# Ced3-han/PepFlowww

Measured on AMD Instinct MI355X. Metric: residues x denoise-steps / s, higher is better.
Workload: dtype f32 (fp32 storage and accumulation; matrix products as 3 x f16 split MFMA, ~22-bit operands); 1 GPU; cfg4/GPU: B=64 x 128-residue synthetic pockets (112 ctx + 16 gen) per GPU; per_gpu_batch=64, residues=128, global_batch=64, parallelism=batch-shard x1, hipgraph=True, precision=fp32

## Files before the change

pepflowww_amd/csrc/ipa_split.hip:

```cpp
#include <cstdlib>
#include <type_traits>
#include "common.h"
#include "../../include/pepflow_hip.h"

#ifdef PF_PROFILE
__device__ long long g_prof_ipas[64];
#define PROFS(i) do { if (blockIdx.x == gridDim.x / 2 + 3 && threadIdx.x == 64) g_prof_ipas[i] = clock64(); } while (0)
extern "C" int pf_debug_prof_ipas(long long* out, int n) {
    return (int)hipMemcpyFromSymbol(out, HIP_SYMBOL(g_prof_ipas), sizeof(long long) * n, 0, hipMemcpyDeviceToHost);
}
#else
#define PROFS(i)
#endif

namespace {

typedef float f32x2 __attribute__((ext_vector_type(2)));
constexpr int H = PF_HEADS, C = PF_C_HID, PQ = PF_QK_PTS, PV = PF_V_PTS;
constexpr int OFF_KV = 1024;
#ifndef PF_IPA_WMAX
#define PF_IPA_WMAX 8
#endif
constexpr int WMAX = PF_IPA_WMAX;
constexpr int KPS = 28;
constexpr int VPS = 36;

__device__ __forceinline__ float softplusf2(float x) { return x > 20.f ? x : log1pf(expf(x)); }

template <bool D16> struct DzVec { typedef float4 type; };
template <> struct DzVec<true> { typedef half4 type; };

template <int NB4, bool D16>
__device__ __forceinline__ void pair_dz_rows(const void* __restrict__ dzp, size_t rowb, int L, int i0, int Le, int kt,
                                             const float* __restrict__ Pw, int SLD, int ks, int cq, f32x2 (&acc)[32]) {
    typedef typename DzVec<D16>::type V4;
    typedef typename std::conditional<D16, _Float16, float>::type DT;
    constexpr int NT = 4 * NB4;
    const DT* base = reinterpret_cast<const DT*>(dzp) + rowb * (size_t)L * 16 + 4 * cq;
    int koff[NT];
    float on[NT];
#pragma unroll
    for (int u = 0; u < NT; ++u) {
        const int uu = min(u, kt - 1);
        koff[u] = min(16 * uu + ks, L - 1) * 16;
        on[u] = u < kt ? 1.f : 0.f;
    }
    auto load_row = [&](int qi, V4 (&buf)[NT]) {
        const DT* row = base + (size_t)min(i0 + qi, Le - 1) * L * 16;
#pragma unroll
        for (int u = 0; u < NT; ++u) buf[u] = *reinterpret_cast<const V4*>(row + koff[u]);
    };
    auto mac_row = [&](int qi, const V4 (&buf)[NT]) {
        const float* pr = Pw + qi * SLD;
#pragma unroll
        for (int u = 0; u < NT; ++u) {
            float pv;
            if (u <= 4 * (NB4 - 1)) pv = pr[16 * u];
            else pv = pr[16 * min(u, kt - 1)] * on[u];
            const f32x2 p2 = {pv, pv};
            f32x2 d0, d1;
            if constexpr (D16) { d0 = (f32x2){(float)buf[u][0], (float)buf[u][1]}; d1 = (f32x2){(float)buf[u][2], (float)buf[u][3]}; }
            else { d0 = (f32x2){buf[u].x, buf[u].y}; d1 = (f32x2){buf[u].z, buf[u].w}; }
            acc[2 * qi] = __builtin_elementwise_fma(d0, p2, acc[2 * qi]);
            acc[2 * qi + 1] = __builtin_elementwise_fma(d1, p2, acc[2 * qi + 1]);
        }
    };
    constexpr int D = NB4 == 1 ? 8 : NB4 == 2 ? 4 : 2;
    V4 buf[D][NT];
#pragma unroll
    for (int d = 0; d < D - 1; ++d) load_row(d, buf[d]);
#pragma unroll
    for (int qi = 0; qi < 16; ++qi) {
        load_row(min(qi + D - 1, 15), buf[(qi + D - 1) % D]);
        __builtin_amdgcn_sched_barrier(0);
        mac_row(qi, buf[qi % D]);
        __builtin_amdgcn_sched_barrier(0);
    }
}

template <bool D16>
__device__ __forceinline__ void pair_dz_phase(const pf_ipa_attn_args& a, size_t rowb, int h, int i0, int Le, int kt, const float* Pwave,
                                              int SLD, float inv, int lane) {
    const int ks = (lane & 3) | ((lane >> 4) << 2), cq = (lane >> 2) & 3;
    f32x2 acc[32];
#pragma unroll
    for (int k = 0; k < 32; ++k) acc[k] = (f32x2){0.f, 0.f};
    const float* Pw = Pwave + ks;
    const int nb4 = (kt + 3) >> 2;
    if (nb4 <= 1) pair_dz_rows<1, D16>(a.dz, rowb, a.L, i0, Le, kt, Pw, SLD, ks, cq, acc);
    else if (nb4 == 2) pair_dz_rows<2, D16>(a.dz, rowb, a.L, i0, Le, kt, Pw, SLD, ks, cq, acc);
    else if (nb4 == 3) pair_dz_rows<3, D16>(a.dz, rowb, a.L, i0, Le, kt, Pw, SLD, ks, cq, acc);
    else pair_dz_rows<4, D16>(a.dz, rowb, a.L, i0, Le, kt, Pw, SLD, ks, cq, acc);
    float v[64];
#pragma unroll
    for (int k = 0; k < 32; ++k) { v[2 * k] = acc[k][0]; v[2 * k + 1] = acc[k][1]; }
    float w[32], x[16], y[8], z4[4];
#pragma unroll
    for (int k = 0; k < 32; ++k) {
        auto rr = __builtin_amdgcn_permlane32_swap(__float_as_uint(v[k]), __float_as_uint(v[k + 32]), false, false);
        w[k] = __uint_as_float(rr[0]) + __uint_as_float(rr[1]);
    }
#pragma unroll
    for (int k = 0; k < 16; ++k) {
        auto rr = __builtin_amdgcn_permlane16_swap(__float_as_uint(w[k]), __float_as_uint(w[k + 16]), false, false);
        x[k] = __uint_as_float(rr[0]) + __uint_as_float(rr[1]);
    }
    {
        const bool hi = lane & 2;
#pragma unroll
        for (int k = 0; k < 8; ++k) {
            const float send = hi ? x[k] : x[k + 8], keep = hi ? x[k + 8] : x[k];
            y[k] = keep + lane_xor2(send);
        }
    }
    {
        const bool hi = lane & 1;
#pragma unroll
        for (int k = 0; k < 4; ++k) {
            const float send = hi ? y[k] : y[k + 4], keep = hi ? y[k + 4] : y[k];
            z4[k] = keep + lane_xor1(send);
        }
    }
    const int qi = ((lane >> 5) & 1) * 8 + ((lane >> 4) & 1) * 4 + (lane & 3);
    const float invq = __shfl(inv, qi);
    const float4 bd = *reinterpret_cast<const float4*>(a.b_dz + 4 * cq);
    const int i = min(i0 + qi, Le - 1);
    *reinterpret_cast<float4*>(a.feats + (rowb + i) * PF_IPA_FEATS + 1408 + h * 16 + 4 * cq) =
        make_float4(z4[0] * invq + bd.x, z4[1] * invq + bd.y, z4[2] * invq + bd.z, z4[3] * invq + bd.w);
}

template <int I, int N, class F> __device__ __forceinline__ void cfor_p(F&& f) {
    if constexpr (I < N) {
        f(std::integral_constant<int, I>{});
        cfor_p<I + 1, N>(f);
    }
}
constexpr int PJ_TILES = 31;
constexpr int PJ_NPAD = 3968;
constexpr int PJ_CT = 3;
constexpr int PJ_NCH = (PJ_TILES + PJ_CT - 1) / PJ_CT;
constexpr int PJ_CHUNK_B = PJ_CT * 8 * 1024;
constexpr int PJ_NB = 4;
constexpr int PJ_STAGE_B = PJ_NB * PJ_CHUNK_B;
__device__ __forceinline__ constexpr int pj_tile(int idx, int h) {
    return idx < 8 ? 8 * h + idx : idx < 24 ? 64 + 16 * h + (idx - 8) : idx < 26 ? 192 + 2 * h + (idx - 24) : 208 + 5 * h + (idx - 26);
}
__device__ __forceinline__ void pj_glds16(const void* sbase, unsigned voff, unsigned lds_addr) {
    const unsigned long long v = (unsigned long long)sbase;
    const unsigned lo = __builtin_amdgcn_readfirstlane((unsigned)v), hi = __builtin_amdgcn_readfirstlane((unsigned)(v >> 32));
    const void* sb = (const void*)(((unsigned long long)hi << 32) | lo);
    lds_addr = __builtin_amdgcn_readfirstlane(lds_addr);
    asm volatile("s_mov_b32 m0, %2\n\ts_nop 4\n\tglobal_load_lds_dwordx4 %0, %1" : : "v"(voff), "s"(sb), "s"(lds_addr) : "memory", "m0");
}
template <int N> __device__ __forceinline__ void pj_wait_vm() { asm volatile("s_waitcnt vmcnt(%0)" : : "n"(N) : "memory"); }
__device__ __forceinline__ void pj_wait_vm_dyn(int n) {
    n = __builtin_amdgcn_readfirstlane(n);
    switch (n > 40 ? 40 : n) {
#define PJ_W(k) case k: pj_wait_vm<k>(); break;
        PJ_W(0) PJ_W(1) PJ_W(2) PJ_W(3) PJ_W(4) PJ_W(5) PJ_W(6) PJ_W(7) PJ_W(8) PJ_W(9) PJ_W(10) PJ_W(11) PJ_W(12) PJ_W(13) PJ_W(14)
        PJ_W(15) PJ_W(16) PJ_W(17) PJ_W(18) PJ_W(19) PJ_W(20) PJ_W(21) PJ_W(22) PJ_W(23) PJ_W(24) PJ_W(25) PJ_W(26) PJ_W(27) PJ_W(28)
        PJ_W(29) PJ_W(30) PJ_W(31) PJ_W(32) PJ_W(33) PJ_W(34) PJ_W(35) PJ_W(36) PJ_W(37) PJ_W(38) PJ_W(39) PJ_W(40)
#undef PJ_W
    }
}
__device__ __forceinline__ constexpr int pj_vt_row(int f) { return f < 64 ? 16 * (f & 3) + (f >> 2) : 64 + 16 * ((f - 64) & 3) + ((f - 64) >> 2); }
__device__ __forceinline__ int pj_vt_pos(int j) { return (j & ~31) + 8 * ((j >> 2) & 3) + 4 * ((j >> 4) & 1) + (j & 3); }
__host__ __device__ __forceinline__ constexpr int pj_vtl(int LP) { return ((LP + 31) & ~31) + 8; }
__host__ __device__ __forceinline__ constexpr int pj_vp_floats(int LP) {
    return LP * VPS > 48 * pj_vtl(LP) ? LP * VPS : 48 * pj_vtl(LP);
}
struct PjW { half8 h[4], l[4]; };
template <bool KF> __device__ __forceinline__ constexpr int pj_ntiles() { return KF ? PJ_TILES - 8 : PJ_TILES; }
template <bool KF> __device__ __forceinline__ constexpr int pj_nch() { return (pj_ntiles<KF>() + PJ_CT - 1) / PJ_CT; }
template <bool KF> __device__ __forceinline__ constexpr int pj_orig(int j) { return KF && j >= 8 ? j + 8 : j; }
__device__ __forceinline__ constexpr bool pj_q_tile(int idx) { return idx < 8 || idx == 24 || idx == 25; }
template <bool KS, bool KF = false>
__device__ __forceinline__ void proj_head(const pf_ipa_attn_args& a, size_t rowb, int iq, int h, int jrow, int LPe, bool wave_on, int role, int tile, float* KP,
                                          _Float16* VPT , int VTL, _Float16* VTH , int VTG,
                                          unsigned char* WS , float* QPW ,
                                          float* PB ,
                                          float4 (&qf)[8], float4 (&qp4)[6], int lane, int wave, int nw) {
    const int r = lane & 15, g = lane >> 4;
    PROFS(8);
    const unsigned char* whp = reinterpret_cast<const unsigned char*>(a.proj_w_f16);
    const unsigned char* wlp = whp + (size_t)PJ_NPAD * 128 * 2;
    const unsigned ws0 = (unsigned)(size_t)(__attribute__((address_space(3))) void*)WS;
    const unsigned l16 = lane * 16;
    const int ppw = (PJ_CT * 8 + nw - 1) / nw;
    constexpr int NT = pj_ntiles<KF>(), NCH = pj_nch<KF>();
    auto issue = [&](int c) __attribute__((always_inline)) {
        const int npc = min(PJ_CT, NT - PJ_CT * c) * 8;
        for (int k = 0; k < ppw; ++k) {
            const int pc = min(wave + k * nw, npc - 1);
            const int tl = pc >> 3, ks = (pc >> 1) & 3, pl = pc & 1;
            const int T16 = pj_tile(pj_orig<KF>(PJ_CT * c + tl), h);
            pj_glds16((pl ? wlp : whp) + (size_t)(T16 * 4 + ks) * 1024, l16, ws0 + (c % PJ_NB) * PJ_CHUNK_B + pc * 1024);
        }
    };
    for (int i = wave * 64 + lane; i < PJ_TILES * 16; i += nw * 64) PB[i] = a.proj_bias[16 * pj_tile(i >> 4, h) + (i & 15)];
    for (int i = wave * 64 + lane; i < 24 * VTL; i += nw * 64) reinterpret_cast<float2*>(VPT)[i] = make_float2(0.f, 0.f);
    PROFS(30);
    half8 xh[4], xl[4];
    float R[9], T[3];
    {
        const float* xrow = a.s_in + (rowb + iq) * 128 + 8 * g;
        float4 t[8];
#pragma unroll
        for (int ks = 0; ks < 4; ++ks) { t[2 * ks] = *reinterpret_cast<const float4*>(xrow + 32 * ks); t[2 * ks + 1] = *reinterpret_cast<const float4*>(xrow + 32 * ks + 4); }
        const float* Rg = a.rot + (rowb + iq) * 9;
        const float* Tg = a.trans + (rowb + iq) * 3;
#pragma unroll
        for (int k = 0; k < 9; ++k) R[k] = Rg[k];
#pragma unroll
        for (int k = 0; k < 3; ++k) T[k] = Tg[k];
#pragma unroll
        for (int ks = 0; ks < 4; ++ks) {
            const float v0[4] = {t[2 * ks].x, t[2 * ks].y, t[2 * ks].z, t[2 * ks].w}, v1[4] = {t[2 * ks + 1].x, t[2 * ks + 1].y, t[2 * ks + 1].z, t[2 * ks + 1].w};
            half4 h0, l0, h1, l1;
            split4(v0, h0, l0);
            split4(v1, h1, l1);
#pragma unroll
            for (int e = 0; e < 4; ++e) { xh[ks][e] = h0[e]; xh[ks][4 + e] = h1[e]; xl[ks][e] = l0[e]; xl[ks][4 + e] = l1[e]; }
        }
    }
    PROFS(31);
    if constexpr (KF && !KS) {
        float* kfrag32 = reinterpret_cast<float*>(VTH + (size_t)8 * (VTG >> 5) * 1024 + (size_t)tile * 4096);
        if (wave_on && role != 1) {
            const float* krow = a.s_in + (rowb + iq) * 128 + 4 * g;
#pragma unroll
            for (int hb = 0; hb < 2; ++hb) {
                float4 kt[4];
#pragma unroll
                for (int u = 0; u < 4; ++u) kt[u] = *reinterpret_cast<const float4*>(krow + 16 * (4 * hb + u));
#pragma unroll
                for (int u = 0; u < 4; ++u) *reinterpret_cast<float4*>(kfrag32 + (4 * hb + u) * 256 + lane * 4) = kt[u];
            }
        }
    }
    PROFS(32);
    asm volatile("" ::: "memory");
#pragma unroll
    for (int c = 0; c < PJ_NB - 1; ++c)
        if (c < NCH) issue(c);
    PROFS(33);
    _Float16* kfrag = VTH + (size_t)8 * (VTG >> 5) * 1024 + (size_t)tile * 4096 + lane * 8;
    float qpr[2][3] = {{0.f, 0.f, 0.f}, {0.f, 0.f, 0.f}};
    auto ldfrag = [&](int c, int tl, PjW& w) __attribute__((always_inline)) {
        const unsigned char* b = WS + (c % PJ_NB) * PJ_CHUNK_B + tl * 8192 + lane * 16;
#pragma unroll
        for (int ks = 0; ks < 4; ++ks) {
            w.h[ks] = *reinterpret_cast<const half8*>(b + ks * 2048);
            w.l[ks] = *reinterpret_cast<const half8*>(b + ks * 2048 + 1024);
        }
    };
    cfor_p<0, NCH>([&](auto ic) __attribute__((always_inline)) {
        constexpr int c = decltype(ic)::value;
        constexpr int NDY = (c + 1 < NCH) + (PJ_NB > 3 && c + 2 < NCH) + (PJ_NB > 4 && c + 3 < NCH);
        static_assert(PJ_NB == 2 || PJ_NB == 4, "wait accounting written for 2 or 4 staging buffers");
        PROFS(9 + 2 * c);
        pj_wait_vm_dyn(PJ_NB == 2 ? 0 : NDY * ppw);
        if constexpr (c == 0) asm volatile("s_waitcnt lgkmcnt(0)" ::: "memory");
        __builtin_amdgcn_s_barrier();
        PROFS(10 + 2 * c);
        asm volatile("" ::: "memory");
        if constexpr (c + PJ_NB - 1 < NCH) issue(c + PJ_NB - 1);
        if (wave_on) {
            PjW wa, wb;
            if (role == 0) ldfrag(c, 0, wa);
            cfor_p<0, PJ_CT>([&](auto it) __attribute__((always_inline)) {
                constexpr int tl = decltype(it)::value, jt = PJ_CT * c + tl, idx = pj_orig<KF>(jt);
                if constexpr (jt < NT) {
                  if (role == 0 || (role == 1) == pj_q_tile(idx)) {
                    PjW& w = (tl & 1) ? wb : wa;
                    if (role != 0) ldfrag(c, tl, w);
                    else if constexpr (tl + 1 < PJ_CT && jt + 1 < NT) ldfrag(c, tl + 1, (tl & 1) ? wa : wb);
                    constexpr bool VTILE = idx >= 16 && idx < 24;
                    f32x4 am = {0.f, 0.f, 0.f, 0.f}, ac = {0.f, 0.f, 0.f, 0.f};
#pragma unroll
                    for (int ks = 0; ks < 4; ++ks) {
                        if constexpr (VTILE) {
                            am = mfma_h(xh[ks], w.h[ks], am);
                            ac = mfma_h(xl[ks], w.h[ks], ac);
                            ac = mfma_h(xh[ks], w.l[ks], ac);
                        } else {
                            am = mfma_h(w.h[ks], xh[ks], am);
                            ac = mfma_h(w.h[ks], xl[ks], ac);
// ... 224 lines not shown
                for (int cc = 0; cc < 3; ++cc) qv[3 * (4 * t2 + gs) + cc] = __shfl(qpr[t2][cc], r + 16 * gs, 64);
#pragma unroll
        for (int q = 0; q < 6; ++q) qp4[q] = make_float4(qv[4 * q], qv[4 * q + 1], qv[4 * q + 2], qv[4 * q + 3]);
    }
}

template <bool VEC4, bool FUSE = false, bool PROJ = false, bool KFRAG = false, bool KF = false, bool HELP = true>
__global__ __launch_bounds__(512) void ipa_scores_kernel(pf_ipa_attn_args a, int nrb, int rows_per_block, int LP, int SLD, unsigned kfs_b ) {
    extern __shared__ __attribute__((aligned(16))) float smem[];
    constexpr bool KSPLIT = PROJ && !FUSE;
    const int L = a.L;
    float* KP = smem;
    float* MJ = KP + LP * KPS;
    float* VP = MJ + LP;
    float* SW = VP + (PROJ ? pj_vp_floats(LP) : LP * VPS);

    const int tid = threadIdx.x, wave = tid >> 6, lane = tid & 63;
    const int r = lane & 15, g = lane >> 4;
    const int lid = xcd_remap(blockIdx.x, gridDim.x);
    const int rb = lid % nrb;
    const int h = (lid / nrb) % H;
    const int b = lid / (nrb * H);
    const size_t rowb = (size_t)b * L;
    const int ntq = rows_per_block >> 4;
    const bool helper = PROJ && HELP && wave >= ntq;
    const int i0 = rb * rows_per_block + (helper ? wave - ntq : wave) * 16;
    const int Le = a.key_end ? min(__builtin_amdgcn_readfirstlane(a.key_end[b]), L) : L;
    const int kt = (Le + 15) >> 4, ktf = Le >> 4;
    const bool wave_on = i0 < Le;
    if (rb * rows_per_block >= Le) return;
    const int LPe = 16 * kt;
    PROFS(0);

    const int iq = max(min(i0 + r, Le - 1), 0);
    float4 qf[8];
    float4 qp4[6];
    if constexpr (!PROJ) {
        const float* qrow = a.proj + (rowb + iq) * a.ldp + h * C + 4 * g;
#pragma unroll
        for (int s = 0; s < 8; ++s) qf[s] = *reinterpret_cast<const float4*>(qrow + 16 * s);
#pragma unroll
        for (int q = 0; q < 6; ++q) qp4[q] = *reinterpret_cast<const float4*>(a.qp + (rowb + iq) * 192 + h * 24 + 4 * q);
    }
    const float mi = a.mask[rowb + iq];
    const float gamma = softplusf2(a.head_w[h]) * 0.09622504486493763f;
    const float* kbase = a.proj + rowb * a.ldp + OFF_KV + h * 2 * C + 4 * g;
    const char* kfr_u = nullptr;
    if constexpr (KSPLIT && KF) {
        kfr_u = reinterpret_cast<const char*>(a.k_frag_s) + (size_t)b * kfs_b;
    } else if constexpr (PROJ) {
        const int VTG = (L + 31) & ~31;
        kfr_u = reinterpret_cast<const char*>(a.att_vt) + (((size_t)b * H + h) * 512 * VTG + (size_t)8 * (VTG >> 5) * 1024) * sizeof(_Float16);
    }
    auto loadk = [&](int t, float4 (&kf)[8]) {
        if constexpr (KSPLIT) {
            const char* kt_u = kfr_u + (size_t)t * 8192;
#pragma unroll
            for (int s = 0; s < 4; ++s) {
                kf[s] = *reinterpret_cast<const float4*>(kt_u + s * 2048 + (unsigned)lane * 16u);
                kf[4 + s] = *reinterpret_cast<const float4*>(kt_u + s * 2048 + 1024 + (unsigned)lane * 16u);
            }
        } else if constexpr (PROJ) {
            const char* kt_u = kfr_u + (size_t)t * 8192;
#pragma unroll
            for (int s = 0; s < 8; ++s) kf[s] = *reinterpret_cast<const float4*>(kt_u + s * 1024 + (unsigned)lane * 16u);
        } else if constexpr (KFRAG) {
            const float* kt_f = a.k_frag + ((((size_t)b * H + h) * (L >> 4) + t) * 8) * 256 + lane * 4;
#pragma unroll
            for (int s = 0; s < 8; ++s) kf[s] = *reinterpret_cast<const float4*>(kt_f + s * 256);
        } else {
            const float* krow = kbase + (size_t)min(16 * t + r, Le - 1) * a.ldp;
#pragma unroll
            for (int s = 0; s < 8; ++s) kf[s] = *reinterpret_cast<const float4*>(krow + 16 * s);
        }
    };
    float4 kf[8], kn[8];
    half8 qh[4], ql[4];
    if constexpr (!PROJ) { if (wave_on) loadk(0, kf); }

    if constexpr (PROJ) {
        for (int j = tid; j < LPe; j += blockDim.x) MJ[j] = j < L ? a.mask[rowb + min(j, L - 1)] : 0.f;
        unsigned char* WS = reinterpret_cast<unsigned char*>(SW);
        float* QPW = reinterpret_cast<float*>(WS + PJ_STAGE_B) + (helper ? 0 : wave) * 16 * 24;
        float* PB = reinterpret_cast<float*>(WS + PJ_STAGE_B) + ntq * 16 * 24;
        const int role = HELP ? ((int)(blockDim.x >> 6) > ntq ? (helper ? 2 : 1) : 0) : 0;
        const int VTG = (L + 31) & ~31;
        _Float16* VTH = reinterpret_cast<_Float16*>(const_cast<void*>(a.att_vt)) + ((size_t)b * H + h) * 512 * VTG;
        proj_head<KSPLIT, KF>(a, rowb, iq, h, i0 + r, LPe, wave_on, role, helper ? wave - ntq : wave, KP, reinterpret_cast<_Float16*>(VP), pj_vtl(LP), VTH, VTG, WS, QPW,
                  PB, qf, qp4, lane, wave, (int)(blockDim.x >> 6));
        __syncthreads();
        if (!wave_on || helper) return;
        loadk(0, kf);
#pragma unroll
        for (int s = 0; KSPLIT && s < 4; ++s) {
            const float v[8] = {qf[2 * s].x, qf[2 * s].y, qf[2 * s].z, qf[2 * s].w, qf[2 * s + 1].x, qf[2 * s + 1].y, qf[2 * s + 1].z, qf[2 * s + 1].w};
#pragma unroll
            for (int j = 0; j < 8; ++j) qh[s][j] = (_Float16)v[j];
            pf_pin(qh[s]);
#pragma unroll
            for (int j = 0; j < 8; ++j) ql[s][j] = (_Float16)(v[j] - (float)qh[s][j]);
        }
    } else {
    {
        const int nth = blockDim.x;
        constexpr int KB = 2, VB = 3;
        float4 k4[KB], v4[VB];
        float mj0 = 0.f;
#pragma unroll
        for (int u = 0; u < KB; ++u) {
            const int idx = min(tid + u * nth, LPe * 6 - 1), j = idx / 6, q = idx - j * 6;
            k4[u] = *reinterpret_cast<const float4*>(a.kp + (rowb + min(j, L - 1)) * 192 + h * 24 + 4 * q);
        }
        mj0 = a.mask[rowb + min(tid, L - 1)];
        mj0 = tid < L ? mj0 : 0.f;
#pragma unroll
        for (int u = 0; u < VB; ++u) {
            const int idx = min(tid + u * nth, LPe * 9 - 1), j = idx / 9, q = idx - j * 9;
            v4[u] = *reinterpret_cast<const float4*>(a.vp + (rowb + min(j, L - 1)) * 288 + h * 36 + 4 * q);
        }
        asm volatile("" : "+v"(k4[0].x), "+v"(k4[0].y), "+v"(k4[0].z), "+v"(k4[0].w), "+v"(k4[1].x), "+v"(k4[1].y), "+v"(k4[1].z), "+v"(k4[1].w), "+v"(mj0));
        asm volatile("" : "+v"(v4[0].x), "+v"(v4[0].y), "+v"(v4[0].z), "+v"(v4[0].w), "+v"(v4[1].x), "+v"(v4[1].y), "+v"(v4[1].z), "+v"(v4[1].w),
                          "+v"(v4[2].x), "+v"(v4[2].y), "+v"(v4[2].z), "+v"(v4[2].w));
#pragma unroll
        for (int u = 0; u < KB; ++u) {
            const int idx = tid + u * nth, j = idx / 6, q = idx - j * 6;
            if (idx < LPe * 6) *reinterpret_cast<float4*>(KP + j * KPS + 4 * q) = k4[u];
        }
        if (tid < LPe) MJ[tid] = mj0;
#pragma unroll
        for (int u = 0; u < VB; ++u) {
            const int idx = tid + u * nth, j = idx / 9, q = idx - j * 9;
            if (idx < LPe * 9) *reinterpret_cast<float4*>(VP + j * VPS + 4 * q) = v4[u];
        }
        for (int idx = tid + KB * nth; idx < LPe * 6; idx += nth) {
            const int j = idx / 6, q = idx - j * 6;
            const float4 v = *reinterpret_cast<const float4*>(a.kp + (rowb + min(j, L - 1)) * 192 + h * 24 + 4 * q);
            *reinterpret_cast<float4*>(KP + j * KPS + 4 * q) = v;
        }
        for (int j = tid + nth; j < LPe; j += nth) MJ[j] = j < L ? a.mask[rowb + j] : 0.f;
        for (int idx = tid + VB * nth; idx < LPe * 9; idx += nth) {
            const int j = idx / 9, q = idx - j * 9;
            *reinterpret_cast<float4*>(VP + j * VPS + 4 * q) = *reinterpret_cast<const float4*>(a.vp + (rowb + min(j, L - 1)) * 288 + h * 36 + 4 * q);
        }
    }
    __syncthreads();
    if (!wave_on) return;
    }
    PROFS(1);

    const float scale_qk = 0.051031036307982884f;
    const float* brow = a.bias + (((size_t)b * H + h) * L + iq) * L;
    float* srow = SW + (size_t)wave * 16 * SLD + r * SLD + 4 * g;
    float mx = -3.0e38f;
    auto qk_tile = [&](int t, const float4 (&kf)[8], auto tail) {
        constexpr bool TAIL = decltype(tail)::value;
        const int jb = 16 * t + 4 * g;
        float bj[4];
        if constexpr (VEC4 && !TAIL) {
            const float4 bv = *reinterpret_cast<const float4*>(brow + jb);
            bj[0] = bv.x; bj[1] = bv.y; bj[2] = bv.z; bj[3] = bv.w;
        } else {
#pragma unroll
            for (int e = 0; e < 4; ++e) bj[e] = brow[TAIL ? min(jb + e, L - 1) : jb + e];
        }
        f32x4 acc = {0.f, 0.f, 0.f, 0.f}, acc2 = {0.f, 0.f, 0.f, 0.f};
        if constexpr (KSPLIT) {
#pragma unroll
            for (int s = 0; s < 4; ++s) {
                const half8 kh = __builtin_bit_cast(half8, kf[s]), kl = __builtin_bit_cast(half8, kf[4 + s]);
                acc = mfma_h(kh, qh[s], acc);
                acc2 = mfma_h(kh, ql[s], acc2);
                acc2 = mfma_h(kl, qh[s], acc2);
            }
        } else {
#pragma unroll
            for (int s = 0; s < 8; s += 2) {
                acc = mfma16(kf[s].x, qf[s].x, acc);   acc2 = mfma16(kf[s + 1].x, qf[s + 1].x, acc2);
                acc = mfma16(kf[s].y, qf[s].y, acc);   acc2 = mfma16(kf[s + 1].y, qf[s + 1].y, acc2);
                acc = mfma16(kf[s].z, qf[s].z, acc);   acc2 = mfma16(kf[s + 1].z, qf[s + 1].z, acc2);
                acc = mfma16(kf[s].w, qf[s].w, acc);   acc2 = mfma16(kf[s + 1].w, qf[s + 1].w, acc2);
            }
        }
        acc += acc2;
        float sv[4];
#pragma unroll
        for (int e = 0; e < 4; ++e) {
            const int j = jb + e;
            const float* kp = KP + j * KPS;
            f32x2 d2 = {0.f, 0.f};
#pragma unroll
            for (int q = 0; q < 6; ++q) {
                const float4 kq = *reinterpret_cast<const float4*>(kp + 4 * q);
                const f32x2 da = (f32x2){qp4[q].x, qp4[q].y} - (f32x2){kq.x, kq.y};
                const f32x2 db = (f32x2){qp4[q].z, qp4[q].w} - (f32x2){kq.z, kq.w};
                d2 = __builtin_elementwise_fma(da, da, d2);
                d2 = __builtin_elementwise_fma(db, db, d2);
            }
            float v = acc[e] * scale_qk + bj[e];
            v = v + (-0.5f) * (gamma * (d2[0] + d2[1]));
            v = v + 1e5f * (mi * MJ[j] - 1.f);
            if constexpr (TAIL) v = j < Le ? v : -3.0e38f;
            sv[e] = v;
            mx = fmaxf(mx, v);
        }
        *reinterpret_cast<float4*>(srow + 16 * t) = make_float4(sv[0], sv[1], sv[2], sv[3]);
    };
    int t = 0;
    for (; t + 1 < ktf; t += 2) {
        loadk(t + 1, kn);
        qk_tile(t, kf, std::false_type{});
        loadk(min(t + 2, kt - 1), kf);
        qk_tile(t + 1, kn, std::false_type{});
    }
    if (ktf & 1) {
        loadk(kt - 1, kn);
        qk_tile(ktf - 1, kf, std::false_type{});
        if (kt > ktf) qk_tile(ktf, kn, std::true_type{});
    } else if (kt > ktf) {
        qk_tile(ktf, kf, std::true_type{});
    }
    PROFS(2);
    mx = max_xor32(max_xor16(mx));
    float sum = 0.f;
    for (int t = 0; t < kt; ++t) {
        float4 v = *reinterpret_cast<const float4*>(srow + 16 * t);
        v.x = exp_softmax(v.x - mx); v.y = exp_softmax(v.y - mx); v.z = exp_softmax(v.z - mx); v.w = exp_softmax(v.w - mx);
        sum += v.x; sum += v.y; sum += v.z; sum += v.w;
        *reinterpret_cast<float4*>(srow + 16 * t) = v;
    }
    sum = sum_xor32(sum_xor16(sum));
    const float inv = 1.f / sum;
    PROFS(3);
    if constexpr (FUSE) {
        asm volatile("s_waitcnt lgkmcnt(0)" ::: "memory");
        __builtin_amdgcn_wave_barrier();
        pair_dz_phase<false>(a, rowb, h, i0, Le, kt, SW + (size_t)wave * 16 * SLD, SLD, inv, lane);
    }
    PROFS(7);
    float* prow = FUSE ? nullptr : a.p_out + (((size_t)b * H + h) * L + iq) * L;

    constexpr int NTC = 11;
    f32x4 O[NTC];
#pragma unroll
    for (int n = 0; n < NTC; ++n) O[n] = (f32x4){0.f, 0.f, 0.f, 0.f};
    if constexpr (PROJ) {
        const int VTG = (L + 31) & ~31, VTL = pj_vtl(LP);
        const char* vt_u = reinterpret_cast<const char*>(a.att_vt) + ((size_t)b * H + h) * 512 * VTG * sizeof(_Float16);
        const unsigned vt_lane = (unsigned)lane * 16u;
        const _Float16* vpt = reinterpret_cast<const _Float16*>(VP) + r * VTL + 8 * g;
        const int steps = (kt + 1) >> 1;
        auto loadv16 = [&](int st, half8 (&vh)[8], half8 (&vl)[8]) {
            const char* su = vt_u + (size_t)st * 2048;
            const size_t tstride = (size_t)(VTG >> 5) * 2048;
#pragma unroll
            for (int n = 0; n < 8; ++n) {
                vh[n] = *reinterpret_cast<const half8*>(su + n * tstride + vt_lane);
                vl[n] = *reinterpret_cast<const half8*>(su + n * tstride + vt_lane + 1024);
            }
        };
        auto pv_step = [&](int st, const half8 (&vh)[8], const half8 (&vl)[8]) {
            const int t0 = 2 * st, t1 = 2 * st + 1;
            float4 p0 = *reinterpret_cast<const float4*>(srow + 16 * t0);
            float4 p1 = *reinterpret_cast<const float4*>(srow + 16 * min(t1, kt - 1));
            p0.x *= inv; p0.y *= inv; p0.z *= inv; p0.w *= inv;
            p1.x *= inv; p1.y *= inv; p1.z *= inv; p1.w *= inv;
            if (t1 >= kt) p1 = make_float4(0.f, 0.f, 0.f, 0.f);
            if constexpr (!FUSE) {
                auto put = [&](int t, const float4& p) {
                    const int jb = 16 * t + 4 * g;
                    if (16 * t + 16 <= Le) {
                        *reinterpret_cast<float4*>(prow + jb) = p;
                    } else {
                        if (jb < Le) prow[jb] = p.x;
                        if (jb + 1 < Le) prow[jb + 1] = p.y;
                        if (jb + 2 < Le) prow[jb + 2] = p.z;
                        if (jb + 3 < Le) prow[jb + 3] = p.w;
                    }
                };
                put(t0, p0);
                if (t1 < kt) put(t1, p1);
            }
            const float pv[8] = {p0.x, p0.y, p0.z, p0.w, p1.x, p1.y, p1.z, p1.w};
            half8 ph, pl;
#pragma unroll
            for (int j = 0; j < 8; ++j) ph[j] = (_Float16)pv[j];
            pf_pin(ph);
#pragma unroll
            for (int j = 0; j < 8; ++j) pl[j] = (_Float16)(pv[j] - (float)ph[j]);
            half8 qh[3], ql[3];
#pragma unroll
            for (int n = 0; n < 3; ++n) {
                qh[n] = *reinterpret_cast<const half8*>(vpt + (16 * n) * VTL + 32 * st);
                ql[n] = *reinterpret_cast<const half8*>(vpt + (48 + 16 * n) * VTL + 32 * st);
            }
#pragma unroll
            for (int n = 0; n < 8; ++n) O[n] = mfma_h(ph, vh[n], O[n]);
#pragma unroll
            for (int n = 0; n < 3; ++n) O[8 + n] = mfma_h(ph, qh[n], O[8 + n]);
#pragma unroll
            for (int n = 0; n < 8; ++n) O[n] = mfma_h(ph, vl[n], O[n]);
#pragma unroll
            for (int n = 0; n < 3; ++n) O[8 + n] = mfma_h(ph, ql[n], O[8 + n]);
#pragma unroll
            for (int n = 0; n < 8; ++n) O[n] = mfma_h(pl, vh[n], O[n]);
#pragma unroll
            for (int n = 0; n < 3; ++n) O[8 + n] = mfma_h(pl, qh[n], O[8 + n]);
        };
        if constexpr (FUSE) {
            half8 va[8], vc[8];
            for (int st = 0; st < steps; ++st) {
                loadv16(st, va, vc);
                pv_step(st, va, vc);
            }
        } else {
            half8 va[8], vc[8], wa[8], wc[8];
            loadv16(0, va, vc);
            int st = 0;
            for (; st + 1 < steps; st += 2) {
                loadv16(st + 1, wa, wc);
                pv_step(st, va, vc);
                loadv16(min(st + 2, steps - 1), va, vc);
                pv_step(st + 1, wa, wc);
            }
            if (steps & 1) pv_step(steps - 1, va, vc);
        }
    } else {
    const float* vbase = a.proj + rowb * a.ldp + OFF_KV + h * 2 * C + C + 4 * r;
        const float* vp0 = VP + r;
        const float* vp2 = VP + (r < 4 ? 32 + r : 0);
        auto loadv = [&](int t, float (&vb)[NTC][4]) {
#pragma unroll
            for (int tt = 0; tt < 4; ++tt) {
                const int j = min(16 * t + 4 * g + tt, Le - 1);
                const float* vrow = vbase + (size_t)j * a.ldp;
                const float4 x = *reinterpret_cast<const float4*>(vrow), y = *reinterpret_cast<const float4*>(vrow + 64);
                vb[0][tt] = x.x; vb[1][tt] = x.y; vb[2][tt] = x.z; vb[3][tt] = x.w;
                vb[4][tt] = y.x; vb[5][tt] = y.y; vb[6][tt] = y.z; vb[7][tt] = y.w;
                vb[8][tt] = vp0[j * VPS]; vb[9][tt] = vp0[j * VPS + 16]; vb[10][tt] = vp2[j * VPS];
            }
        };
        float vb[NTC][4], vn[NTC][4];
        loadv(0, vb);
        auto pv_tile = [&](int t, const float (&vb)[NTC][4], auto tail) {
            constexpr bool TAIL = decltype(tail)::value;
            float4 p = *reinterpret_cast<const float4*>(srow + 16 * t);
            p.x *= inv; p.y *= inv; p.z *= inv; p.w *= inv;
            const int jb = 16 * t + 4 * g;
            if constexpr (FUSE) {
            } else if constexpr (VEC4 && !TAIL) {
                *reinterpret_cast<float4*>(prow + jb) = p;
            } else if constexpr (!TAIL) {
                prow[jb] = p.x; prow[jb + 1] = p.y; prow[jb + 2] = p.z; prow[jb + 3] = p.w;
            } else {
                if (jb < Le) prow[jb] = p.x;
                if (jb + 1 < Le) prow[jb + 1] = p.y;
                if (jb + 2 < Le) prow[jb + 2] = p.z;
                if (jb + 3 < Le) prow[jb + 3] = p.w;
            }
#pragma unroll
            for (int n = 0; n < NTC; ++n) O[n] = mfma16(p.x, vb[n][0], O[n]);
#pragma unroll
            for (int n = 0; n < NTC; ++n) O[n] = mfma16(p.y, vb[n][1], O[n]);
#pragma unroll
            for (int n = 0; n < NTC; ++n) O[n] = mfma16(p.z, vb[n][2], O[n]);
#pragma unroll
            for (int n = 0; n < NTC; ++n) O[n] = mfma16(p.w, vb[n][3], O[n]);
        };
        for (t = 0; t + 1 < ktf; t += 2) {
            loadv(t + 1, vn);
            pv_tile(t, vb, std::false_type{});
            loadv(min(t + 2, kt - 1), vb);
            pv_tile(t + 1, vn, std::false_type{});
        }
        if (ktf & 1) {
            loadv(kt - 1, vn);
            pv_tile(ktf - 1, vb, std::false_type{});
            if (kt > ktf) pv_tile(ktf, vn, std::true_type{});
        } else if (kt > ktf) {
            pv_tile(ktf, vb, std::true_type{});
        }
    }
    PROFS(4);
    float* opt = SW + (size_t)wave * 16 * SLD;
#pragma unroll
    for (int e = 0; e < 4; ++e) {
        const int ti = 4 * g + e, i = min(i0 + ti, Le - 1);
        float* f = a.feats + (rowb + i) * PF_IPA_FEATS + h * C + 4 * r;
        *reinterpret_cast<float4*>(f) = make_float4(O[0][e], O[1][e], O[2][e], O[3][e]);
        *reinterpret_cast<float4*>(f + 64) = make_float4(O[4][e], O[5][e], O[6][e], O[7][e]);
        opt[ti * 36 + r] = O[8][e];
        opt[ti * 36 + 16 + r] = O[9][e];
        if (r < 4) opt[ti * 36 + 32 + r] = O[10][e];
    }
    asm volatile("s_waitcnt lgkmcnt(0)" ::: "memory");
    __builtin_amdgcn_wave_barrier();
    PROFS(5);
    for (int idx = lane; idx < 16 * PV; idx += 64) {
        const int ti = idx / PV, p = idx - ti * PV;
        const int i = min(i0 + ti, Le - 1);
        const float* R = a.rot + (rowb + i) * 9;
        const float* T = a.trans + (rowb + i) * 3;
        const float* o = opt + ti * 36 + p * 3;
        const float x = o[0] - T[0], y = o[1] - T[1], z = o[2] - T[2];
        const float lx = R[0] * x + R[3] * y + R[6] * z;
        const float ly = R[1] * x + R[4] * y + R[7] * z;
        const float lz = R[2] * x + R[5] * y + R[8] * z;
        float* f = a.feats + (rowb + i) * PF_IPA_FEATS + h * PV + p;
        f[1024] = lx;
        f[1120] = ly;
        f[1216] = lz;
        f[1312] = sqrtf(lx * lx + ly * ly + lz * lz + 1e-8f);
    }
    PROFS(6);
}

template <bool FUSE = false, bool PROJ = false, bool KF = false>
__global__ __launch_bounds__(512) void ipa_scores16_kernel(pf_ipa_attn_args a, int nrb, int rows_per_block, int SLD) {
    extern __shared__ __attribute__((aligned(16))) float smem[];
    const int L = a.L;
    float* KP = smem;
    float* MJ = KP + L * KPS;
    float* SW = MJ + L;
    const int VTS = ((L + 31) & ~31) + 8;
    const int sw_floats = PROJ ? max((int)(blockDim.x >> 6) * 16 * SLD, (int)((PJ16_STAGE_B + (blockDim.x >> 6) * 1536 + PJ_TILES * 64) / 4)) : 0;
    _Float16* KL = reinterpret_cast<_Float16*>(SW + sw_floats);
    _Float16* VT = KL + L * KLS;

    const int tid = threadIdx.x, wave = tid >> 6, lane = tid & 63;
    const int r = lane & 15, g = lane >> 4;
    const int lid = xcd_remap(blockIdx.x, gridDim.x);
    const int rb = lid % nrb;
    const int h = (lid / nrb) % H;
    const int b = lid / (nrb * H);
    const size_t rowb = (size_t)b * L;
    const int i0 = rb * rows_per_block + wave * 16;
    const int LK = a.key_end ? min((__builtin_amdgcn_readfirstlane(a.key_end[b]) + 15) & ~15, L) : L;
    const int L32 = (LK + 31) & ~31;
    const int kt = LK >> 4;
    const bool wave_on = i0 < LK;
    if (rb * rows_per_block >= LK) return;
    const int iq = i0 + r;
    PROFS(0);

    constexpr int RS = 1024;
    const _Float16* qk = reinterpret_cast<const _Float16*>(a.att_qk);
    auto ldfrag = [&](const _Float16* row, int c0, int s, half8& fh) { fh = *reinterpret_cast<const half8*>(row + c0 + 32 * s + 8 * g); };
    half8 qh[4];
    float4 qp4[6];
    if constexpr (!PROJ) {
        const _Float16* qrow = qk + (rowb + (wave_on ? iq : 0)) * RS;
#pragma unroll
        for (int s4 = 0; s4 < 4; ++s4) ldfrag(qrow, h * C, s4, qh[s4]);
#pragma unroll
        for (int q = 0; q < 6; ++q) qp4[q] = *reinterpret_cast<const float4*>(a.qp + (rowb + (wave_on ? iq : 0)) * 192 + h * 24 + 4 * q);
    }
    const float mi = a.mask[rowb + (wave_on ? iq : 0)];
    const float gamma = softplusf2(a.head_w[h]) * 0.09622504486493763f;
    auto loadk = [&](int t, half8 (&kh)[4]) {
        if constexpr (PROJ) {
            const _Float16* krow = KL + (16 * t + r) * KLS + 8 * g;
#pragma unroll
            for (int s4 = 0; s4 < 4; ++s4) kh[s4] = *reinterpret_cast<const half8*>(krow + 32 * s4);
        } else {
            const _Float16* kb = qk + (size_t)a.B * L * 1024 + ((((size_t)b * H + h) * (L >> 4) + t) * 4) * 512 + lane * 8;
#pragma unroll
            for (int s4 = 0; s4 < 4; ++s4) kh[s4] = *reinterpret_cast<const half8*>(kb + s4 * 512);
        }
    };
    half8 kh[4], nh[4];
    if constexpr (!PROJ) { if (wave_on) loadk(0, kh); }

    if constexpr (PROJ) {
        for (int j = tid; j < LK; j += blockDim.x) MJ[j] = a.mask[rowb + j];
        for (int idx = tid; idx < PF_ATT_VROWS * (L32 - LK); idx += blockDim.x) {
            const int row = idx / (L32 - LK), col = LK + idx - row * (L32 - LK);
            VT[row * VTS + col] = (_Float16)0.f;
        }
        unsigned char* WS = reinterpret_cast<unsigned char*>(SW);
        float* QPW = reinterpret_cast<float*>(WS + PJ16_STAGE_B) + wave * (1536 / 4);
        float* PB = reinterpret_cast<float*>(WS + PJ16_STAGE_B) + (blockDim.x >> 6) * (1536 / 4);
        proj_head16<KF>(a, rowb, wave_on ? iq : 0, h, i0 + r, wave_on, KP, KL, VT, VTS, WS, QPW, PB, qh, qp4, lane, wave, (int)(blockDim.x >> 6));
        __syncthreads();
        if (!wave_on) return;
        loadk(0, kh);
    } else {

    {
        const int nth = blockDim.x;
        constexpr int KB = 6;
        float4 k4[KB];
#pragma unroll
        for (int u = 0; u < KB; ++u) {
            const int idx = min(tid + u * nth, max(LK * 6 - 1, 0)), j = idx / 6, q = idx - j * 6;
            k4[u] = *reinterpret_cast<const float4*>(a.kp + (rowb + j) * 192 + h * 24 + 4 * q);
        }
        float mj0 = a.mask[rowb + min(tid, max(LK - 1, 0))];
        asm volatile("" : "+v"(k4[0].x), "+v"(k4[0].y), "+v"(k4[0].z), "+v"(k4[0].w), "+v"(k4[1].x), "+v"(k4[1].y), "+v"(k4[1].z), "+v"(k4[1].w),
                          "+v"(k4[2].x), "+v"(k4[2].y), "+v"(k4[2].z), "+v"(k4[2].w), "+v"(mj0));
        asm volatile("" : "+v"(k4[3].x), "+v"(k4[3].y), "+v"(k4[3].z), "+v"(k4[3].w), "+v"(k4[4].x), "+v"(k4[4].y), "+v"(k4[4].z), "+v"(k4[4].w),
                          "+v"(k4[5].x), "+v"(k4[5].y), "+v"(k4[5].z), "+v"(k4[5].w));
#pragma unroll
        for (int u = 0; u < KB; ++u) {
            const int idx = tid + u * nth, j = idx / 6, q = idx - j * 6;
            if (idx < LK * 6) *reinterpret_cast<float4*>(KP + j * KPS + 4 * q) = k4[u];
        }
        if (tid < LK) MJ[tid] = mj0;
        for (int idx = tid + KB * nth; idx < LK * 6; idx += nth) {
            const int j = idx / 6, q = idx - j * 6;
            *reinterpret_cast<float4*>(KP + j * KPS + 4 * q) = *reinterpret_cast<const float4*>(a.kp + (rowb + j) * 192 + h * 24 + 4 * q);
        }
        for (int j = tid + nth; j < LK; j += nth) MJ[j] = a.mask[rowb + j];
    }
    __syncthreads();
    if (!wave_on) return;
    }
    PROFS(1);

    const float scale_qk = 0.051031036307982884f;
    const float* brow = a.bias + (((size_t)b * H + h) * L + iq) * L;
    float* srow = SW + (size_t)wave * 16 * SLD + r * SLD;
    float mx = -3.0e38f;
    auto qk_tile = [&](int t, const half8 (&kh)[4], const float4& bv) {
        const int jb = 16 * t + 4 * g;
        const float bj[4] = {bv.x, bv.y, bv.z, bv.w};
        f32x4 am = {0.f, 0.f, 0.f, 0.f};
#pragma unroll
        for (int s4 = 0; s4 < 4; ++s4) am = mfma_h(kh[s4], qh[s4], am);
        float sv[4];
#pragma unroll
        for (int e = 0; e < 4; ++e) {
            const int j = jb + e;
            const float* kp = KP + j * KPS;
            f32x2 d2 = {0.f, 0.f};
#pragma unroll
            for (int q = 0; q < 6; ++q) {
                const float4 kq = *reinterpret_cast<const float4*>(kp + 4 * q);
// ... 604 lines not shown
```

Measured before the change: 2.972 million res*step/s.

## Keep IPA attention scores in registers for KSPLIT path with nested unrolled pipeline

For the KSPLIT variant, the QK score tiles now stay in a register array instead of being written to and re-read from LDS. Softmax is applied in registers, the probabilities are written straight to global memory, and they are fed directly into the PV MFMAs. The QK and PV loops are fully unrolled with a compile-time bounded nest (at most 8 or 4 tiles), with explicit sched_barriers and split loading of the V high/low planes. This cuts LDS traffic and waits but raises register pressure, and it relies on kt being at most MAXT.

```diff
diff --git a/pepflowww_amd/csrc/ipa_split.hip b/pepflowww_amd/csrc/ipa_split.hip
--- a/pepflowww_amd/csrc/ipa_split.hip
+++ b/pepflowww_amd/csrc/ipa_split.hip
@@ -133,6 +133,14 @@
     if constexpr (I < N) {
         f(std::integral_constant<int, I>{});
         cfor_p<I + 1, N>(f);
+    }
+}
+template <int I, int N, class F> __device__ __forceinline__ void nest_p(int n, F&& f) {
+    if constexpr (I < N) {
+        if (I == 0 || n > I) {
+            f(std::integral_constant<int, I>{});
+            nest_p<I + 1, N>(n, f);
+        }
     }
 }
 constexpr int PJ_TILES = 31;
@@ -663,7 +671,7 @@
     const float* brow = a.bias + (((size_t)b * H + h) * L + iq) * L;
     float* srow = SW + (size_t)wave * 16 * SLD + r * SLD + 4 * g;
     float mx = -3.0e38f;
-    auto qk_tile = [&](int t, const float4 (&kf)[8], auto tail) {
+    auto qk_tile = [&](int t, const float4 (&kf)[8], auto tail, float4& out) __attribute__((always_inline)) {
         constexpr bool TAIL = decltype(tail)::value;
         const int jb = 16 * t + 4 * g;
         float bj[4];
@@ -714,21 +722,28 @@
             sv[e] = v;
             mx = fmaxf(mx, v);
         }
-        *reinterpret_cast<float4*>(srow + 16 * t) = make_float4(sv[0], sv[1], sv[2], sv[3]);
+        out = make_float4(sv[0], sv[1], sv[2], sv[3]);
+    };
+    auto qk_tile_lds = [&](int t, const float4 (&kf)[8], auto tail) {
+        float4 s4;
+        qk_tile(t, kf, tail, s4);
+        *reinterpret_cast<float4*>(srow + 16 * t) = s4;
     };
     int t = 0;
+    float inv;
+    if constexpr (!KSPLIT) {
     for (; t + 1 < ktf; t += 2) {
         loadk(t + 1, kn);
-        qk_tile(t, kf, std::false_type{});
+        qk_tile_lds(t, kf, std::false_type{});
         loadk(min(t + 2, kt - 1), kf);
-        qk_tile(t + 1, kn, std::false_type{});
+        qk_tile_lds(t + 1, kn, std::false_type{});
     }
     if (ktf & 1) {
         loadk(kt - 1, kn);
-        qk_tile(ktf - 1, kf, std::false_type{});
-        if (kt > ktf) qk_tile(ktf, kn, std::true_type{});
+        qk_tile_lds(ktf - 1, kf, std::false_type{});
+        if (kt > ktf) qk_tile_lds(ktf, kn, std::true_type{});
     } else if (kt > ktf) {
-        qk_tile(ktf, kf, std::true_type{});
+        qk_tile_lds(ktf, kf, std::true_type{});
     }
     PROFS(2);
     mx = max_xor32(max_xor16(mx));
@@ -740,57 +755,54 @@
         *reinterpret_cast<float4*>(srow + 16 * t) = v;
     }
     sum = sum_xor32(sum_xor16(sum));
-    const float inv = 1.f / sum;
-    PROFS(3);
+    inv = 1.f / sum;
+    }
+    if constexpr (!KSPLIT) PROFS(3);
     if constexpr (FUSE) {
         asm volatile("s_waitcnt lgkmcnt(0)" ::: "memory");
         __builtin_amdgcn_wave_barrier();
         pair_dz_phase<false>(a, rowb, h, i0, Le, kt, SW + (size_t)wave * 16 * SLD, SLD, inv, lane);
     }
-    PROFS(7);
+    if constexpr (!KSPLIT) PROFS(7);
     float* prow = FUSE ? nullptr : a.p_out + (((size_t)b * H + h) * L + iq) * L;
 
     constexpr int NTC = 11;
     f32x4 O[NTC];
-#pragma unroll
-    for (int n = 0; n < NTC; ++n) O[n] = (f32x4){0.f, 0.f, 0.f, 0.f};
+    if constexpr (!KSPLIT) {
+#pragma unroll
+        for (int n = 0; n < NTC; ++n) O[n] = (f32x4){0.f, 0.f, 0.f, 0.f};
+    }
     if constexpr (PROJ) {
         const int VTG = (L + 31) & ~31, VTL = pj_vtl(LP);
         const char* vt_u = reinterpret_cast<const char*>(a.att_vt) + ((size_t)b * H + h) * 512 * VTG * sizeof(_Float16);
         const unsigned vt_lane = (unsigned)lane * 16u;
         const _Float16* vpt = reinterpret_cast<const _Float16*>(VP) + r * VTL + 8 * g;
         const int steps = (kt + 1) >> 1;
+        const size_t tstride = (size_t)(VTG >> 5) * 2048;
+        auto loadvp = [&](int st, int plane, half8 (&v)[8]) __attribute__((always_inline)) {
+            const char* su = vt_u + (size_t)st * 2048 + plane * 1024;
+            unsigned vo = vt_lane;
+            asm volatile("" : "+v"(vo));
+#pragma unroll
+            for (int n = 0; n < 8; ++n) v[n] = *reinterpret_cast<const half8*>(su + n * tstride + vo);
+        };
         auto loadv16 = [&](int st, half8 (&vh)[8], half8 (&vl)[8]) {
             const char* su = vt_u + (size_t)st * 2048;
-            const size_t tstride = (size_t)(VTG >> 5) * 2048;
 #pragma unroll
             for (int n = 0; n < 8; ++n) {
                 vh[n] = *reinterpret_cast<const half8*>(su + n * tstride + vt_lane);
                 vl[n] = *reinterpret_cast<const half8*>(su + n * tstride + vt_lane + 1024);
             }
         };
-        auto pv_step = [&](int st, const half8 (&vh)[8], const half8 (&vl)[8]) {
-            const int t0 = 2 * st, t1 = 2 * st + 1;
-            float4 p0 = *reinterpret_cast<const float4*>(srow + 16 * t0);
-            float4 p1 = *reinterpret_cast<const float4*>(srow + 16 * min(t1, kt - 1));
-            p0.x *= inv; p0.y *= inv; p0.z *= inv; p0.w *= inv;
-            p1.x *= inv; p1.y *= inv; p1.z *= inv; p1.w *= inv;
-            if (t1 >= kt) p1 = make_float4(0.f, 0.f, 0.f, 0.f);
-            if constexpr (!FUSE) {
-                auto put = [&](int t, const float4& p) {
-                    const int jb = 16 * t + 4 * g;
-                    if (16 * t + 16 <= Le) {
-                        *reinterpret_cast<float4*>(prow + jb) = p;
-                    } else {
-                        if (jb < Le) prow[jb] = p.x;
-                        if (jb + 1 < Le) prow[jb + 1] = p.y;
-                        if (jb + 2 < Le) prow[jb + 2] = p.z;
-                        if (jb + 3 < Le) prow[jb + 3] = p.w;
-                    }
-                };
-                put(t0, p0);
-                if (t1 < kt) put(t1, p1);
-            }
+        auto put = [&](int t, const float4& p) __attribute__((always_inline)) { *reinterpret_cast<float4*>(prow + 16 * t + 4 * g) = p; };
+        auto put_tail = [&](int t, const float4& p) __attribute__((always_inline)) {
+            const int jb = 16 * t + 4 * g;
+            if (jb < Le) prow[jb] = p.x;
+            if (jb + 1 < Le) prow[jb + 1] = p.y;
+            if (jb + 2 < Le) prow[jb + 2] = p.z;
+            if (jb + 3 < Le) prow[jb + 3] = p.w;
+        };
+        auto pv_mma = [&](int st, const float4& p0, const float4& p1, const half8 (&vh)[8], const half8 (&vl)[8], auto lo_done) __attribute__((always_inline)) {
             const float pv[8] = {p0.x, p0.y, p0.z, p0.w, p1.x, p1.y, p1.z, p1.w};
             half8 ph, pl;
 #pragma unroll
@@ -812,6 +824,7 @@
             for (int n = 0; n < 8; ++n) O[n] = mfma_h(ph, vl[n], O[n]);
 #pragma unroll
             for (int n = 0; n < 3; ++n) O[8 + n] = mfma_h(ph, ql[n], O[8 + n]);
+            lo_done();
 #pragma unroll
             for (int n = 0; n < 8; ++n) O[n] = mfma_h(pl, vh[n], O[n]);
 #pragma unroll
@@ -821,19 +834,66 @@
             half8 va[8], vc[8];
             for (int st = 0; st < steps; ++st) {
                 loadv16(st, va, vc);
-                pv_step(st, va, vc);
+                const int t1 = 2 * st + 1;
+                float4 p0 = *reinterpret_cast<const float4*>(srow + 32 * st);
+                float4 p1 = *reinterpret_cast<const float4*>(srow + 16 * min(t1, kt - 1));
+                p0.x *= inv; p0.y *= inv; p0.z *= inv; p0.w *= inv;
+                p1.x *= inv; p1.y *= inv; p1.z *= inv; p1.w *= inv;
+                if (t1 >= kt) p1 = make_float4(0.f, 0.f, 0.f, 0.f);
+                pv_mma(st, p0, p1, va, vc, [] {});
             }
         } else {
-            half8 va[8], vc[8], wa[8], wc[8];
-            loadv16(0, va, vc);
-            int st = 0;
-            for (; st + 1 < steps; st += 2) {
-                loadv16(st + 1, wa, wc);
-                pv_step(st, va, vc);
-                loadv16(min(st + 2, steps - 1), va, vc);
-                pv_step(st + 1, wa, wc);
-            }
-            if (steps & 1) pv_step(steps - 1, va, vc);
+            constexpr int MAXT = HELP ? 4 : 8;
+            float4 sc[MAXT];
+#pragma unroll
+            for (int tc = 0; tc < MAXT; ++tc) sc[tc] = make_float4(-3.0e38f, -3.0e38f, -3.0e38f, -3.0e38f);
+            nest_p<0, MAXT>(kt, [&](auto it) __attribute__((always_inline)) {
+                constexpr int tc = decltype(it)::value;
+                __builtin_amdgcn_sched_barrier(0);
+                if constexpr (tc + 1 < MAXT) loadk(min(tc + 1, kt - 1), (tc & 1) ? kf : kn);
+                const float4 (&kc)[8] = (tc & 1) ? kn : kf;
+                if (Le >= 16 * (tc + 1)) qk_tile(tc, kc, std::false_type{}, sc[tc]);
+                else qk_tile(tc, kc, std::true_type{}, sc[tc]);
+            });
+            half8 va[8], wa[8], vc[8];
+            __builtin_amdgcn_sched_barrier(0);
+            loadvp(0, 0, va);
+            loadvp(0, 1, vc);
+            __builtin_amdgcn_sched_barrier(0);
+            PROFS(2);
+            mx = max_xor32(max_xor16(mx));
+            float sum = 0.f;
+#pragma unroll
+            for (int tc = 0; tc < MAXT; ++tc) {
+                float4 v = sc[tc];
+                v.x = exp_softmax(v.x - mx); v.y = exp_softmax(v.y - mx); v.z = exp_softmax(v.z - mx); v.w = exp_softmax(v.w - mx);
+                sum += v.x; sum += v.y; sum += v.z; sum += v.w;
+                sc[tc] = v;
+            }
+            sum = sum_xor32(sum_xor16(sum));
+            inv = 1.f / sum;
+            PROFS(3);
+#pragma unroll
+            for (int tc = 0; tc < MAXT; ++tc) {
+                sc[tc].x *= inv; sc[tc].y *= inv; sc[tc].z *= inv; sc[tc].w *= inv;
+                if (16 * tc + 16 <= Le) put(tc, sc[tc]);
+                else if (16 * tc < Le) put_tail(tc, sc[tc]);
+            }
+            PROFS(7);
+#pragma unroll
+            for (int n = 0; n < NTC; ++n) O[n] = (f32x4){0.f, 0.f, 0.f, 0.f};
+            nest_p<0, MAXT / 2>(steps, [&](auto is) __attribute__((always_inline)) {
+                constexpr int st = decltype(is)::value;
+                __builtin_amdgcn_sched_barrier(0);
+                if constexpr (st + 1 < MAXT / 2) loadvp(min(st + 1, steps - 1), 0, (st & 1) ? va : wa);
+                pv_mma(st, sc[2 * st], sc[2 * st + 1], (st & 1) ? wa : va, vc, [&]() __attribute__((always_inline)) {
+                    if constexpr (st + 1 < MAXT / 2) {
+                        __builtin_amdgcn_sched_barrier(0);
+                        loadvp(min(st + 1, steps - 1), 1, vc);
+                        __builtin_amdgcn_sched_barrier(0);
+                    }
+                });
+            });
         }
     } else {
     const float* vbase = a.proj + rowb * a.ldp + OFF_KV + h * 2 * C + C + 4 * r;
@@ -892,7 +952,7 @@
         }
     }
     PROFS(4);
-    float* opt = SW + (size_t)wave * 16 * SLD;
+    float* opt = SW + (size_t)wave * 16 * (KSPLIT ? 36 : SLD);
 #pragma unroll
     for (int e = 0; e < 4; ++e) {
         const int ti = 4 * g + e, i = min(i0 + ti, Le - 1);
```

Result: faster. 3.014 million res*step/s, median of 6 (+1.4%).
